# mmSir/SpatioTemporalEntropyModel

Hardware: AMD Instinct MI355X
Metric: frames/s (higher is better)
Workload: dtype f32; 1 GPU; configs[1]: SpatioTemporalPriorModel_Res(256,192) training step on mbt2018(192,192) latents, 16 septuplets x 7 frames x 256x256 per GPU, EMLoss, clip 1.0 + Adam 1e-4 / aux Adam 1e-3; per_gpu_batch=16, global_batch=16, parallelism=dp1, stream_priorities=latents=0,side=-1,compute=-1, stream_cu_masks=latents=block:160, plan_selectors=library defaults

## Files before the change

spatiotemporalentropymodel_amd/_lib.py:

```python
from __future__ import annotations

import ctypes as C
import os

from . import _abi

_PKG = os.path.dirname(os.path.abspath(__file__))
HIP_SO = os.environ.get("STEM_HIP_LIBRARY") or os.path.join(_PKG, "libstem_hip.so")
RANS_SO = os.environ.get("STEM_RANS_LIBRARY") or os.path.join(_PKG, "libstem_rans.so")

DP_SO = os.environ.get("STEM_DP_LIBRARY") or os.path.join(_PKG, "libstem_dp.so")
_hip = None
_rans = None
_dp = None


class StemLibraryError(RuntimeError):
    pass


def _header(name):
    path = os.path.join(_PKG, "..", "include", name)
    if not os.path.exists(path):
        raise StemLibraryError(f"{path} is missing: the ctypes prototypes and structures are read from the C headers")
    return path


def _tables(header):
    protos = _abi.prototypes(_header(header))
    return protos, {n: args for n, (_, args) in protos.items()}, {n: res for n, (res, _) in protos.items() if res is not C.c_int}


_HIP_PROTO, _HIP_SIG, _RESTYPE = _tables("stem_hip.h")
_HIP_BATCH_PROTO, _HIP_BATCH_SIG, _ = _tables("stem_ar_batch.h")
_HIP_BLOCKS_PROTO, _HIP_BLOCKS_SIG, _ = _tables("stem_blocks.h")
_HIP_HYPERPRIOR_PROTO, _HIP_HYPERPRIOR_SIG, _ = _tables("stem_hyperprior.h")
_RANS_PROTO, _RANS_SIG, _RANS_RESTYPE = _tables("stem_rans.h")
_DP_PROTO, _DP_SIG, _ = _tables("stem_dp.h")
_STRUCTS = _abi.structs(_header("stem_hip.h"))


class PackDesc(C.Structure):
    _fields_ = _STRUCTS["stem_pack_desc"]


class F16PackDesc(C.Structure):
    _fields_ = _STRUCTS["stem_f16x2_pack_desc"]


class F16PairDesc(C.Structure):
    _fields_ = _STRUCTS["stem_f16x2_pair_desc"]


class UnpackDesc(C.Structure):
    _fields_ = _STRUCTS["stem_unpack_desc"]


class BiasFinalDesc(C.Structure):
    _fields_ = _STRUCTS["stem_bias_final_desc"]


class WaveSeg(C.Structure):
    _fields_ = _STRUCTS["stem_wave_seg"]


def _bind(lib, protos):
    for name, (restype, argtypes) in protos.items():
        fn = getattr(lib, name)
        fn.argtypes = argtypes
        fn.restype = restype
    return lib


def hip():
    global _hip
    if _hip is None:
        if not os.path.exists(HIP_SO):
            raise StemLibraryError(
                f"{HIP_SO} is missing: build it with `python -c 'import __graft_entry__ as g; g.build()'` "
                "(hipcc --offload-arch=gfx950).  There is no CPU fallback for the STEM kernels.")
        lib = C.CDLL(HIP_SO)
        for protos in (_HIP_PROTO, _HIP_BATCH_PROTO, _HIP_BLOCKS_PROTO, _HIP_HYPERPRIOR_PROTO):
            _bind(lib, protos)
        _hip = lib
    return _hip


def rans():
    global _rans
    if _rans is None:
        if not os.path.exists(RANS_SO):
            raise StemLibraryError(f"{RANS_SO} is missing: run `make -C {os.path.join(_PKG, 'csrc')}`")
        _rans = _bind(C.CDLL(RANS_SO), _RANS_PROTO)
    return _rans


def check(rc: int):
    if rc != 0:
        raise RuntimeError((hip().stem_last_error() or b"").decode() or f"libstem_hip error {rc}")


def declared_hip_symbols():
    return sorted(_HIP_SIG)


# ... 28 lines not shown
```

spatiotemporalentropymodel_amd/csrc/conv_f16x3.hip:

```cpp
#include <math.h>
#include <stdlib.h>

#include <type_traits>

#include "f16x3_layout.h"

namespace {

constexpr int XP = BN + 4;
constexpr int imax(int a, int b) { return a > b ? a : b; }
constexpr int lds_stages(int depth) { return depth == 3 ? 3 : 2; }
constexpr int lds_taps(int bm, int depth) { return imax(imax(lds_stages(depth) * NPL * (bm + BN) * 64, 6 * NPL * bm * 64 + NPL * BN * 64), bm * XP * 4); }
constexpr int lds_total(int bm, int depth) { return lds_taps(bm, depth) + 32 * 4; }

struct Fx3Phase {
    int ntaps, S;
    int dy0, dx0;
    int wofs;
    int cps, nsplit;
    int wsofs;
    int ooy, oox;
};

struct Fx3Args {
// ... 533 lines not shown
            h16x8 h0, h1;
#pragma unroll
            for (int c = 0; c < 4; ++c) {
                hp_t x0, x1;
                q_split(v0[c], oscale, x0, x1);
                h0[c] = x0; h1[c] = x1;
                q_split(v1[c], oscale, x0, x1);
                h0[4 + c] = x0; h1[4 + c] = x1;
            }
            unsigned char *dst = yp + (size_t)m * opix + sl * SLAB + p * 16;
            *reinterpret_cast<h16x8 *>(dst) = h0;
            *reinterpret_cast<h16x8 *>(dst + 64) = h1;
        }
    }
}

enum { GEN_EPI_BIAS = 0, GEN_EPI_LRELU = 1, GEN_EPI_DACT = 2 };

constexpr int GTP = GBN + 4;
constexpr bool GEN_DEFAULT_MFMA16 = true;
constexpr int glds_main(int gbm) { return 2 * NPL * (gbm + GBN) * 64 > gbm * GTP * 4 ? 2 * NPL * (gbm + GBN) * 64 : gbm * GTP * 4; }
constexpr int glds(int gbm) { return glds_main(gbm) + 32 * 4; }

template <int GBM, int MS, bool PH = false>
__global__ __launch_bounds__(GBM * 4, 2) void conv_f16x3_gen_kernel(const Fx3Args a)
{
    static_assert(MS == 32 || MS == 16, "MFMA shape");
    int bxt = blockIdx.x, phase = 0;
    if constexpr (PH) {
        phase = blockIdx.x / a.ptiles;
        bxt = blockIdx.x - phase * a.ptiles;
    }
    const int ntaps = PH ? a.ph[phase].ntaps : a.ntaps, tapS = PH ? a.ph[phase].S : a.S;
    const int cps = PH ? a.ph[phase].cps : a.cps, nsplit = PH ? a.ph[phase].nsplit : a.nsplit;
    const int pdy0 = PH ? a.ph[phase].dy0 : (int)a.dy[0], pdx0 = PH ? a.ph[phase].dx0 : (int)a.dx[0];
    const int wofs = PH ? a.ph[phase].wofs : 0;
    if constexpr (PH) {
        if ((int)blockIdx.z >= nsplit) return;
    }
    float *const wsb = PH ? a.ws + a.ph[phase].wsofs : a.ws;
    constexpr int GNT = GBM * 4, GA_PLANE = GBM * 64, GA_BUF = NPL * GA_PLANE;
    constexpr int PL = NPL, BPC = NPL * GBN * 4 / GNT;
    extern __shared__ __attribute__((aligned(16))) unsigned char smem[];
    unsigned char *As = smem;
    unsigned char *Bs = smem + 2 * GA_BUF;
    int *tapi = reinterpret_cast<int *>(smem + glds_main(GBM));
// ... 188 lines not shown
            step(1, raB, rbB);
            __syncthreads();
        }
        if (q < q_end) {
            step(0, raA, rbA);
            __syncthreads();
        }
    } else {
        int q = q_begin;
        for (; q + 1 < q_end; q += 2) {
            step_dead(0, raA, rbA);
            __syncthreads();
            step_dead(1, raB, rbB);
            __syncthreads();
        }
        if (q < q_end) {
            step_dead(0, raA, rbA);
            __syncthreads();
        }
    }

    float *T = reinterpret_cast<float *>(smem);
    const int Npad = gridDim.y * GBN;
    constexpr int ERS = GNT / 32, ER = GBM / ERS;
    const int ec4 = tid & 31, er0 = tid >> 5;
    f32x4 ev[ER];
    auto OROW = [&](int m) -> size_t {
        if constexpr (!PH) return (size_t)m;
        const int ohw = a.OH * a.OW, b = m / ohw, rem = m - b * ohw, qy = rem / a.OW, qx = rem - qy * a.OW;
        return ((size_t)b * a.OHf + 2 * qy + a.ph[phase].ooy) * a.OWf + 2 * qx + a.ph[phase].oox;
    };
    auto MOK = [&](int m) -> bool {
        if (m >= Mtot) return false;
        if constexpr (!PH) return true;
        const int ohw = a.OH * a.OW, rem = m % ohw, qy = rem / a.OW, qx = rem - qy * a.OW;
        return 2 * qy + a.ph[phase].ooy < a.OHf && 2 * qx + a.ph[phase].oox < a.OWf;
    };
    if (nsplit > 1) {
        float *wsp = wsb + (size_t)zsplit * Mtot * Npad;
#pragma unroll
        for (int j = 0; j < 2; ++j) {
#pragma unroll
            for (int r = 0; r < 16; ++r) {
                const int m = bm0 + ROWL(r), n = bn0 + COLL(j, r);
                if (m < Mtot) __hip_atomic_store(&wsp[(size_t)m * Npad + n], acc[j][r], __ATOMIC_RELAXED, __HIP_MEMORY_SCOPE_AGENT);
            }
        }
        asm volatile("s_waitcnt vmcnt(0)" ::: "memory");
        __syncthreads();
        if (tid == 0) {
            int *c = a.cnt + blockIdx.y * gridDim.x + blockIdx.x;
            tapi[0] = splitk_last_arriver(c, nsplit);
        }
        __syncthreads();
        if (!tapi[0]) return;
        constexpr int SC1 = 16;
        const __amdgpu_buffer_rsrc_t rws = __builtin_amdgcn_make_buffer_rsrc(wsb, 0, (int)((size_t)nsplit * Mtot * Npad * 4), 0x00020000);
        const int sstep = Mtot * Npad * 4;
        int eoff[ER];
#pragma unroll
        for (int k = 0; k < ER; ++k) {
            const int m = bm0 + er0 + ERS * k;
            eoff[k] = m < Mtot ? (m * Npad + bn0 + ec4 * 4) * 4 : OOR;
        }
#pragma unroll
        for (int k = 0; k < ER; ++k) ev[k] = f32x4{0.f, 0.f, 0.f, 0.f};
#pragma unroll
        for (int kb = 0; kb < ER; kb += 4)
            for (int sp = 0; sp < nsplit; sp += 4) {
                f32x4 tt[4][4];
#pragma unroll
                for (int k = 0; k < 4; ++k)
#pragma unroll
                    for (int u = 0; u < 4; ++u)
                        tt[k][u] = __builtin_bit_cast(f32x4, __builtin_amdgcn_raw_buffer_load_b128(rws, sp + u < nsplit ? eoff[kb + k] : OOR,
                                                                                                      (sp + u < nsplit ? sp + u : 0) * sstep, SC1));
#pragma unroll
                for (int k = 0; k < 4; ++k)
#pragma unroll
                    for (int u = 0; u < 4; ++u) ev[kb + k] += tt[k][u];
            }
    } else {
#pragma unroll
        for (int j = 0; j < 2; ++j)
#pragma unroll
            for (int r = 0; r < 16; ++r) T[ROWL(r) * GTP + COLL(j, r)] = acc[j][r];
        __syncthreads();
#pragma unroll
        for (int k = 0; k < ER; ++k) ev[k] = *reinterpret_cast<const f32x4 *>(&T[(er0 + ERS * k) * GTP + ec4 * 4]);
    }
    float omax = 0.f;
    const int ecol = bn0 + ec4 * 4;
    const bool colok = ecol < a.N;
    f32x4 ebias = {0.f, 0.f, 0.f, 0.f};
    if (a.bias && colok) {
#pragma unroll
        for (int c = 0; c < 4; ++c) ebias[c] = a.bias[ecol + c];
    }
    f32x4 ez[ER];
    if (a.epi == GEN_EPI_DACT) {
#pragma unroll
        for (int k = 0; k < ER; ++k) {
            const int m = bm0 + er0 + ERS * k;
            ez[k] = (colok && MOK(m)) ? *reinterpret_cast<const f32x4 *>(a.z + OROW(m) * a.ldz + ecol) : f32x4{1.f, 1.f, 1.f, 1.f};
        }
    }
#pragma unroll
    for (int k = 0; k < ER; ++k) {
        const int row = er0 + ERS * k, m = bm0 + row;
        f32x4 v = ev[k] * fac + ebias;
        if (a.epi == GEN_EPI_LRELU) {
#pragma unroll
            for (int c = 0; c < 4; ++c) v[c] = v[c] > 0.f ? v[c] : v[c] * a.slope;
        } else if (a.epi == GEN_EPI_DACT) {
#pragma unroll
            for (int c = 0; c < 4; ++c) v[c] = ez[k][c] > 0.f ? v[c] : v[c] * a.slope;
        }
        if (colok && MOK(m)) {
            if (a.y) *reinterpret_cast<f32x4 *>(a.y + OROW(m) * a.ldy + ecol) = v;
            omax = fmaxf(fmaxf(omax, fmaxf(fabsf(v[0]), fabsf(v[1]))), fmaxf(fabsf(v[2]), fabsf(v[3])));
        }
        if (a.yp) *reinterpret_cast<f32x4 *>(&T[row * GTP + ec4 * 4]) = v;
    }
    if (a.yq) {
        omax = block_max(omax, qred);
        if (tid == 0) {
            a.yq[QREC_HDR + blockIdx.y * gridDim.x + blockIdx.x] = omax;
            if (blockIdx.x == 0 && blockIdx.y == 0) {
                q_header(a.yq, gridDim.x * gridDim.y);
                if (!a.yp) a.yq[1] = 1.f;
            }
        }
    }
    if (a.yp) {
        __syncthreads();
        const int oslab = a.N / KC, opix = oslab * SLAB;
        unsigned char *yp = static_cast<unsigned char *>(a.yp);
        for (int e = tid; e < GBM * (GBN / 8); e += GNT) {
            const int row = e / (GBN / 8), c8 = e - row * (GBN / 8);
            const int m = bm0 + row, n = bn0 + c8 * 8;
            if (!MOK(m) || n >= a.N) continue;
            const f32x4 v0 = *reinterpret_cast<const f32x4 *>(&T[row * GTP + c8 * 8]);
            const f32x4 v1 = *reinterpret_cast<const f32x4 *>(&T[row * GTP + c8 * 8 + 4]);
            h16x8 h0, h1;
#pragma unroll
            for (int c = 0; c < 4; ++c) {
                hp_t x0, x1;
                q_split(v0[c], oscale, x0, x1);
                h0[c] = x0; h1[c] = x1;
                q_split(v1[c], oscale, x0, x1);
                h0[4 + c] = x0; h1[4 + c] = x1;
            }
            unsigned char *dst = yp + OROW(m) * opix + (n >> 5) * SLAB + ((n >> 3) & 3) * 16;
            *reinterpret_cast<h16x8 *>(dst) = h0;
            *reinterpret_cast<h16x8 *>(dst + 64) = h1;
        }
    }
}

}

static int conv2d_f16x3_launch(const void *xp, const float *xq, const void *wp, const float *bias, const float *beta, const void *gp,
                                float beta_min, int act, float slope, float *y, int ldy, void *yp, float *yq, int B, int H, int W, int C, int N,
                                int R, int S, int stride, int pad, void *stream);

STEM_EXPORT int stem_conv2d_f16x3_fwd(const void *xp, const float *xq, const void *wp, const float *bias, const float *beta, const void *gp,
                                       float beta_min, float *y, int ldy, void *yp, float *yq, int B, int H, int W, int C, int N, int R, int S,
                                       int stride, int pad, void *stream)
{
    return conv2d_f16x3_launch(xp, xq, wp, bias, beta, gp, beta_min, 0, 0.f, y, ldy, yp, yq, B, H, W, C, N, R, S, stride, pad, stream);
}

STEM_EXPORT int stem_conv2d_f16x3_fwd_act(const void *xp, const float *xq, const void *wp, const float *bias, int act, float slope, float *y, int ldy,
                                           void *yp, float *yq, int B, int H, int W, int C, int N, int R, int S, int stride, int pad, void *stream)
{
    STEM_CHECK_ARG(act == 0 || act == 1, "stem_conv2d_f16x3_fwd_act: act is 0 (none) or 1 (leaky ReLU with `slope`)");
    STEM_CHECK_ARG(!act || fabsf(slope) <= 1.f, "stem_conv2d_f16x3_fwd_act: |slope| <= 1");
    return conv2d_f16x3_launch(xp, xq, wp, bias, nullptr, nullptr, 1e-6f, act, slope, y, ldy, yp, yq, B, H, W, C, N, R, S, stride, pad, stream);
}

// ... 73 lines not shown
    const int forced = stem_tuning(STEM_TUNE_FX3_SPLIT);
    if (forced > 0) return forced < nchunks ? forced : nchunks;
    if (nchunks <= 40 && tiles >= 128) return 1;
    int best = 1;
    double best_cost = 1e30;
    for (int s = 1; s <= 16 && s * 8 <= nchunks; ++s) {
        const int cps = cdiv(nchunks, s), ns = cdiv(nchunks, cps), rounds = cdiv(tiles * ns, 256);
        const double cost = rounds * (cps + 6.0) * (rounds == 1 ? 1.67 : 1.0) + (ns > 1 ? 0.3 * ns : 0.0);
        if (cost < best_cost - 1e-9) {
            best_cost = cost;
            best = ns;
        }
    }
    return best;
}

int gen_bm(int M, int ntn, int nchunks)
{
    const int forced = stem_tuning(STEM_TUNE_FX3_GEN_TILE);
    if (forced) return forced;
    (void)nchunks;
    return cdiv(M, 128) * ntn >= 64 ? 128 : 64;
}
}

STEM_EXPORT size_t stem_conv2d_f16x3_gen_workspace_bytes(int B, int H, int W, int C, int N, int R, int S, int stride, int pad, int taps)
{
    const int OH = (H + 2 * pad - R) / stride + 1, OW = (W + 2 * pad - S) / stride + 1;
    if (OH < 1 || OW < 1 || C % 32) return 0;
    const int M = B * OH * OW, nchunks = (C / 32) * (taps > 0 ? taps : R * S), tiles = cdiv(M, gen_bm(M, cdiv(N, GBN), nchunks)) * cdiv(N, GBN);
    int s = gen_split(tiles, nchunks);
    if (stem_fx3_img_eligible(B, H, W, N, R, S, stride, pad)) {
        const int si = stem_fx3_img_split(stem_fx3_img_tiles(B, H, W, N), nchunks);
        if (si > s) s = si;
    }
    while (s > 1 && (size_t)s * M * cdiv(N, GBN) * GBN * sizeof(float) >= 0x7FFFFF00ull) --s;
    return s > 1 ? kGenCntBytes + (size_t)s * M * cdiv(N, GBN) * GBN * sizeof(float) : 0;
}

STEM_EXPORT int stem_conv2d_f16x3_gen_fwd(const void *xp, const float *xq, int xpix, const void *wp, const float *bias, int epi, float slope,
                                           const float *z, int ldz, float *y, int ldy, void *yp, float *yq, int B, int H, int W, int C, int N, int R,
                                           int S, int stride, int pad, int taps, void *ws, size_t ws_bytes, void *stream)
{
    STEM_CHECK_ARG(taps >= 0 && taps <= R * S, "stem_conv2d_f16x3_gen_fwd: 0 <= taps <= R*S (taps=%d)", taps);
    const int T = taps > 0 ? taps : R * S;
    STEM_CHECK_ARG(xp && xq && wp && (y || yp) && (yq || !yp), "stem_conv2d_f16x3_gen_fwd: null pointer (planes come with their scale records)");
    STEM_CHECK_ARG(epi == GEN_EPI_BIAS || fabsf(slope) <= 1.f, "stem_conv2d_f16x3_gen_fwd: |slope| <= 1");
    STEM_CHECK_ARG(B >= 1 && H >= 1 && W >= 1 && C >= 32 && C % 32 == 0 && N >= 4 && N % 4 == 0 && R >= 1 && S >= 1 && R * S <= MAXTAP &&
                   stride >= 1 && pad >= 0, "stem_conv2d_f16x3_gen_fwd: C %% 32 == 0, N %% 4 == 0, R*S <= %d (C=%d N=%d R=%d S=%d)", MAXTAP, C, N, R, S);
    STEM_CHECK_ARG(!yp || N % 32 == 0, "stem_conv2d_f16x3_gen_fwd: planes output needs N %% 32 == 0 (N=%d)", N);
    STEM_CHECK_ARG(!y || (ldy >= N && ldy % 4 == 0 && ((uintptr_t)y & 15) == 0), "stem_conv2d_f16x3_gen_fwd: y rows must be 16-byte aligned, ldy >= N");
    STEM_CHECK_ARG(epi >= GEN_EPI_BIAS && epi <= GEN_EPI_DACT, "stem_conv2d_f16x3_gen_fwd: unknown epilogue %d", epi);
    STEM_CHECK_ARG(epi != GEN_EPI_DACT || (z && ldz >= N && ldz % 4 == 0 && ((uintptr_t)z & 15) == 0), "stem_conv2d_f16x3_gen_fwd: DACT needs z (16-byte aligned rows)");
    const int OH = (H + 2 * pad - R) / stride + 1, OW = (W + 2 * pad - S) / stride + 1;
    STEM_CHECK_ARG(OH >= 1 && OW >= 1, "stem_conv2d_f16x3_gen_fwd: empty output");
    if (xpix == 0) xpix = (C / 32) * SLAB;
    STEM_CHECK_ARG(xpix >= (C / 32) * SLAB && xpix % SLAB == 0, "stem_conv2d_f16x3_gen_fwd: xpix must be a multiple of %d bytes covering C channels", SLAB);
    const size_t xb = (size_t)B * H * W * xpix, wb = gen_image_bytes(N, C, R, S);
    const int M = B * OH * OW, ntn = cdiv(N, GBN), nchunks = (C / 32) * T, bm = gen_bm(M, ntn, nchunks), tiles = cdiv(M, bm) * ntn;
    STEM_CHECK_ARG(xb < 0x7FFFFF00ull && wb < 0x7FFFFF00ull && (size_t)M * ntn * GBN * 4 < 0x7FFFFF00ull,
                   "stem_conv2d_f16x3_gen_fwd: operand views must stay below 2 GiB (split the batch)");
    Fx3Args a;
    memset(&a, 0, sizeof(a));
    a.xp = xp; a.wp = wp; a.bias = bias; a.y = y; a.yp = yp; a.ldy = ldy; a.z = z; a.ldz = ldz; a.epi = epi; a.slope = slope;
    const float *wq = reinterpret_cast<const float *>(static_cast<const unsigned char *>(wp) + wb);
    a.xq = xq; a.yq = yq; a.wq = wq;
    a.B = B; a.H = H; a.W = W; a.C = C; a.N = N; a.OH = OH; a.OW = OW; a.stride = stride; a.ntaps = T; a.S = S;
    a.xbytes = (int)xb; a.wbytes = (int)wb; a.xpix = xpix;
    for (int r = 0; r < R; ++r)
        for (int s = 0; s < S; ++s) {
            a.dy[r * S + s] = (signed char)(r - pad);
            a.dx[r * S + s] = (signed char)(s - pad);
        }
    const bool img = stem_fx3_img_eligible(B, H, W, N, R, S, stride, pad);
    const int itiles = img ? stem_fx3_img_tiles(B, H, W, N) : 0;
    int split = img ? stem_fx3_img_split(itiles, nchunks) : gen_split(tiles, nchunks);
    while (split > 1 && (size_t)split * M * ntn * GBN * sizeof(float) >= 0x7FFFFF00ull) --split;
    const size_t need = kGenCntBytes + (size_t)split * M * ntn * GBN * sizeof(float);
    if (split > 1 && (!ws || ws_bytes < need || (size_t)tiles * sizeof(int) > kGenCntBytes)) split = 1;
    if (img)
        return stem_fx3_img_launch(xp, xq, xpix, (int)xb, wp, wq, (int)wb,
                                   bias, epi, slope, z, ldz, y, ldy, yp, yq, B, H, W, C, N, R, T, split,
                                   split > 1 ? reinterpret_cast<float *>(static_cast<unsigned char *>(ws) + kGenCntBytes) : nullptr,
                                   split > 1 ? static_cast<int *>(ws) : nullptr, stream);
    a.nsplit = split;
    a.cps = cdiv(nchunks, split);
    a.nsplit = cdiv(nchunks, a.cps);
    if (a.nsplit > 1) {
        a.cnt = static_cast<int *>(ws);
        a.ws = reinterpret_cast<float *>(static_cast<unsigned char *>(ws) + kGenCntBytes);
    }
    static bool attr_done = false;
    if (!attr_done) {
        (void)hipFuncSetAttribute((const void *)conv_f16x3_gen_kernel<64, 32>, hipFuncAttributeMaxDynamicSharedMemorySize, glds(64));
        (void)hipFuncSetAttribute((const void *)conv_f16x3_gen_kernel<128, 32>, hipFuncAttributeMaxDynamicSharedMemorySize, glds(128));
        (void)hipFuncSetAttribute((const void *)conv_f16x3_gen_kernel<64, 16>, hipFuncAttributeMaxDynamicSharedMemorySize, glds(64));
        (void)hipFuncSetAttribute((const void *)conv_f16x3_gen_kernel<128, 16>, hipFuncAttributeMaxDynamicSharedMemorySize, glds(128));
        attr_done = true;
    }
    const dim3 grid(cdiv(M, bm), ntn, a.nsplit);
    const int gmsel = stem_tuning(STEM_TUNE_FX3_GEN_MFMA);
    const bool g16 = gmsel ? gmsel == 16 : GEN_DEFAULT_MFMA16;
    if (bm == 128 && g16)
        hipLaunchKernelGGL((conv_f16x3_gen_kernel<128, 16>), grid, dim3(512), glds(128), (hipStream_t)stream, a);
    else if (bm == 128)
        hipLaunchKernelGGL((conv_f16x3_gen_kernel<128, 32>), grid, dim3(512), glds(128), (hipStream_t)stream, a);
    else if (g16)
        hipLaunchKernelGGL((conv_f16x3_gen_kernel<64, 16>), grid, dim3(256), glds(64), (hipStream_t)stream, a);
    else
        hipLaunchKernelGGL((conv_f16x3_gen_kernel<64, 32>), grid, dim3(256), glds(64), (hipStream_t)stream, a);
    STEM_LAUNCH_CHECK("stem_conv2d_f16x3_gen_fwd");
    return 0;
}

namespace {
int tconv_cps(int tiles_per_phase, const int (&nchunks)[4])
{
    const int forced = stem_tuning(STEM_TUNE_FX3_SPLIT);
    int maxc = 0;
    for (int p = 0; p < 4; ++p) maxc = nchunks[p] > maxc ? nchunks[p] : maxc;
    if (forced > 0) return cdiv(maxc, forced < maxc ? forced : maxc);
    if (stem_tuning(STEM_TUNE_TCONV_CPS) > 0) return stem_tuning(STEM_TUNE_TCONV_CPS);
    for (int cps = 12; cps < maxc; ++cps) {
        int wgs = 0, maxns = 0;
        for (int p = 0; p < 4; ++p) {
            const int ns = cdiv(nchunks[p], cps);
// ... 99 lines not shown
```

spatiotemporalentropymodel_amd/csrc/pack.hip:

```cpp
#include <stdarg.h>

#include "stem_common.h"

static thread_local char g_err[512] = "";
void stem_set_error(const char *fmt, ...)
{
    va_list ap;
    va_start(ap, fmt);
    vsnprintf(g_err, sizeof(g_err), fmt, ap);
    va_end(ap);
}
STEM_EXPORT const char *stem_last_error(void) { return g_err; }
STEM_EXPORT int stem_abi_version(void) { return 5; }

static int g_tuning[STEM_TUNE_COUNT] = {0};
static const char *const kTuningNames[STEM_TUNE_COUNT] = {"fx3_tile", "fx3_split", "wg3_split", "arp_workers", "fx3_depth", "fx3_gen_tile", "fx3_mfma", "fx3_gen_mfma", "fx3_gen_img", "fx3_img_w", "wg3_row", "wg3_minch", "tconv_cps", "arp_giveup_at", "unpack_mb"};
int stem_tuning(int id) { return g_tuning[id]; }
STEM_EXPORT int stem_tuning_set(const char *name, int value)
{
    STEM_CHECK_ARG(name && value >= 0, "stem_tuning_set: null name or negative value");
    for (int i = 0; i < STEM_TUNE_COUNT; ++i)
        if (!strcmp(name, kTuningNames[i])) {
            STEM_CHECK_ARG(i != STEM_TUNE_FX3_TILE || value == 0 || value == 64 || value == 128, "stem_tuning_set: fx3_tile is 0 (automatic), 64 or 128");
            STEM_CHECK_ARG(i != STEM_TUNE_FX3_GEN_TILE || value == 0 || value == 64 || value == 128, "stem_tuning_set: fx3_gen_tile is 0 (automatic), 64 or 128");
            STEM_CHECK_ARG(i != STEM_TUNE_FX3_DEPTH || value == 0 || value == 2 || value == 3, "stem_tuning_set: fx3_depth is 0 (automatic), 2 or 3 (LDS stages of the split-operand main loops)");
            STEM_CHECK_ARG(i != STEM_TUNE_FX3_GEN_MFMA || value == 0 || value == 16 || value == 32, "stem_tuning_set: fx3_gen_mfma is 0 (automatic), 16 or 32 (rows of the general kernel's MFMA shape)");
            STEM_CHECK_ARG(i != STEM_TUNE_UNPACK_MB || value == 0 || (value % 32 == 0 && value >= 32 && value <= 192), "stem_tuning_set: unpack_mb is 0 (automatic) or a multiple of 32 up to 192");
            STEM_CHECK_ARG(i != STEM_TUNE_FX3_MFMA || value == 0 || value == 16 || value == 32, "stem_tuning_set: fx3_mfma is 0 (automatic), 16 or 32 (rows of the MFMA shape)");
            g_tuning[i] = value;
            return 0;
        }
    stem_set_error("stem_tuning_set: unknown selector '%s' (fx3_tile, fx3_split, wg3_split, arp_workers, fx3_depth, fx3_gen_tile, fx3_mfma, fx3_gen_mfma, fx3_gen_img, fx3_img_w, wg3_row, wg3_minch, tconv_cps, arp_giveup_at, unpack_mb)", name);
    return -1;
}
STEM_EXPORT int stem_tuning_get(const char *name)
{
    for (int i = 0; name && i < STEM_TUNE_COUNT; ++i)
        if (!strcmp(name, kTuningNames[i])) return g_tuning[i];
    return -1;
}

namespace {

__global__ __launch_bounds__(256) void pack_kernel(float *w, float *out, int A, int Bd, int T, long sa, long sb,
                                                   int R, int S, int masked)
{
    extern __shared__ float tile[];
    const int a = blockIdx.x;
    const int n = Bd * T;
    for (int i = threadIdx.x; i < n; i += 256) {
        const int b = i / T, t = i - b * T;
        float v = w[a * sa + b * sb + t];
        if (masked & 3) {
            const int r = t / S, s = t - r * S;
            if (r > R / 2 || (r == R / 2 && s >= S / 2 + ((masked >> 2) & 1))) {
// ... 419 lines not shown
```

spatiotemporalentropymodel_amd/csrc/stem_common.h:

```cpp
#pragma once
#include <hip/hip_runtime.h>
#include <stdint.h>
#include <stdio.h>
#include <string.h>

#include "../../include/stem_hip.h"

#define STEM_EXPORT extern "C" __attribute__((visibility("default")))

void stem_set_error(const char *fmt, ...);

#define STEM_CHECK_ARG(cond, ...)        \
    do {                                 \
        if (!(cond)) {                   \
            stem_set_error(__VA_ARGS__); \
            return -1;                   \
        }                                \
    } while (0)

#define STEM_LAUNCH_CHECK(name)                                                         \
    do {                                                                                \
        hipError_t e_ = hipGetLastError();                                              \
        if (e_ != hipSuccess) {                                                         \
            stem_set_error("%s: launch failed: %s", name, hipGetErrorString(e_));       \
            return -2;                                                                  \
        }                                                                               \
    } while (0)

typedef float f32x4 __attribute__((ext_vector_type(4)));
typedef float f32x16 __attribute__((ext_vector_type(16)));

static inline int cdiv(int a, int b) { return (a + b - 1) / b; }
static inline size_t cdivz(size_t a, size_t b) { return (a + b - 1) / b; }

enum { STEM_TUNE_FX3_TILE = 0, STEM_TUNE_FX3_SPLIT, STEM_TUNE_WG3_SPLIT, STEM_TUNE_ARP_WORKERS, STEM_TUNE_FX3_DEPTH, STEM_TUNE_FX3_GEN_TILE, STEM_TUNE_FX3_MFMA, STEM_TUNE_FX3_GEN_MFMA, STEM_TUNE_FX3_GEN_IMG, STEM_TUNE_FX3_IMG_W, STEM_TUNE_WG3_ROW, STEM_TUNE_WG3_MINCH, STEM_TUNE_TCONV_CPS, STEM_TUNE_ARP_GIVEUP_AT, STEM_TUNE_UNPACK_MB, STEM_TUNE_COUNT };
int stem_tuning(int id);
bool stem_fx3_img_eligible(int B, int H, int W, int N, int R, int S, int stride, int pad);
int stem_fx3_img_tiles(int B, int H, int W, int N);
int stem_fx3_img_split(int tiles, int nchunks);
int stem_fx3_img_launch(const void *xp, const float *xq, int xpix, int xbytes, const void *wp, const float *wq, int wbytes, const float *bias, int epi,
                        float slope, const float *z, int ldz, float *y, int ldy, void *yp, float *yq, int B, int H, int W, int C, int N, int KS,
                        int T, int split, float *ws, int *cnt, void *stream);

#define STEM_ADAM_CHUNK 4096

typedef _Float16 hp_t;
typedef hp_t hp8 __attribute__((ext_vector_type(8)));
#define STEM_MFMA16(a, b, c) __builtin_amdgcn_mfma_f32_32x32x16_f16(a, b, c, 0, 0, 0)

constexpr int QREC_HDR = 16;
#ifdef __HIPCC__
__device__ inline int q_nslots(const float *q) { return reinterpret_cast<const int *>(q)[0]; }
__device__ inline float q_inv(const float *q) { return q[1]; }
__device__ inline void q_header(float *q, int n)
{
    reinterpret_cast<int *>(q)[0] = n;
#pragma unroll
    for (int i = 2; i < QREC_HDR; ++i) q[i] = 0.f;
// ... 66 lines not shown
```

Baseline: 10020 frames/s.

## Add pointwise 1x1 conv kernel with four-stage LDS ring and plan selector

Adds a dedicated 1x1, stride-1 kernel for the f16x3 general convolution. It streams activation and weight chunks through a four-slot LDS ring using buffer-to-LDS loads, and uses hand-scheduled 16x16x32 MFMA interleaving with explicit waitcnt and barrier control. The epilogue is factored into shared helpers, and plan selection moves into a gen_plan function that is exported and gated by a new fx3_gen_pw tuning selector. The aim is to hide load latency for pointwise convolutions. The trade-off is a larger LDS footprint, which can lower occupancy, plus more complex synchronisation.

```diff
diff --git a/include/stem_plan.h b/include/stem_plan.h
--- /dev/null
+++ b/include/stem_plan.h
@@ -0,0 +1,16 @@
+#ifndef STEM_PLAN_H
+#define STEM_PLAN_H
+
+#include <stddef.h>
+
+#ifdef __cplusplus
+extern "C" {
+#endif
+
+int stem_conv2d_f16x3_gen_plan(int B, int H, int W, int C, int N, int R, int S, int stride, int pad, int taps, size_t ws_bytes, int *split);
+
+#ifdef __cplusplus
+}
+#endif
+
+#endif
diff --git a/spatiotemporalentropymodel_amd/_lib.py b/spatiotemporalentropymodel_amd/_lib.py
--- a/spatiotemporalentropymodel_amd/_lib.py
+++ b/spatiotemporalentropymodel_amd/_lib.py
@@ -35,6 +35,7 @@
 _HIP_BATCH_PROTO, _HIP_BATCH_SIG, _ = _tables("stem_ar_batch.h")
 _HIP_BLOCKS_PROTO, _HIP_BLOCKS_SIG, _ = _tables("stem_blocks.h")
 _HIP_HYPERPRIOR_PROTO, _HIP_HYPERPRIOR_SIG, _ = _tables("stem_hyperprior.h")
+_HIP_PLAN_PROTO, _HIP_PLAN_SIG, _ = _tables("stem_plan.h")
 _RANS_PROTO, _RANS_SIG, _RANS_RESTYPE = _tables("stem_rans.h")
 _DP_PROTO, _DP_SIG, _ = _tables("stem_dp.h")
 _STRUCTS = _abi.structs(_header("stem_hip.h"))
@@ -80,7 +81,7 @@
                 f"{HIP_SO} is missing: build it with `python -c 'import __graft_entry__ as g; g.build()'` "
                 "(hipcc --offload-arch=gfx950).  There is no CPU fallback for the STEM kernels.")
         lib = C.CDLL(HIP_SO)
-        for protos in (_HIP_PROTO, _HIP_BATCH_PROTO, _HIP_BLOCKS_PROTO, _HIP_HYPERPRIOR_PROTO):
+        for protos in (_HIP_PROTO, _HIP_BATCH_PROTO, _HIP_BLOCKS_PROTO, _HIP_HYPERPRIOR_PROTO, _HIP_PLAN_PROTO):
             _bind(lib, protos)
         _hip = lib
     return _hip
diff --git a/spatiotemporalentropymodel_amd/csrc/conv_f16x3.hip b/spatiotemporalentropymodel_amd/csrc/conv_f16x3.hip
--- a/spatiotemporalentropymodel_amd/csrc/conv_f16x3.hip
+++ b/spatiotemporalentropymodel_amd/csrc/conv_f16x3.hip
@@ -579,6 +579,109 @@
 constexpr int glds_main(int gbm) { return 2 * NPL * (gbm + GBN) * 64 > gbm * GTP * 4 ? 2 * NPL * (gbm + GBN) * 64 : gbm * GTP * 4; }
 constexpr int glds(int gbm) { return glds_main(gbm) + 32 * 4; }
 
+constexpr int GEN_ER = 8;
+template <int GBM, typename TPos>
+__device__ __forceinline__ void gen_park(float *T, TPos tpos, const f32x16 (&acc)[2], f32x4 (&ev)[GEN_ER])
+{
+    constexpr int ERS = GBM * 4 / 32;
+    const int tid = threadIdx.x, ec4 = tid & 31, er0 = tid >> 5;
+#pragma unroll
+    for (int j = 0; j < 2; ++j)
+#pragma unroll
+        for (int r = 0; r < 16; ++r) T[tpos(j, r)] = acc[j][r];
+    __syncthreads();
+#pragma unroll
+    for (int k = 0; k < GEN_ER; ++k) ev[k] = *reinterpret_cast<const f32x4 *>(&T[(er0 + ERS * k) * GTP + ec4 * 4]);
+}
+
+template <int GBM, bool PH>
+__device__ __forceinline__ void gen_epilogue(const Fx3Args &a, const int phase, const int bm0, const int bn0, const float fac, const float oscale,
+                                             float *T, float *qred, const f32x4 (&ev)[GEN_ER])
+{
+    constexpr int GNT = GBM * 4, ERS = GNT / 32, ER = GEN_ER;
+    static_assert(ER * ERS == GBM, "eight pieces per thread");
+    const int tid = threadIdx.x, ec4 = tid & 31, er0 = tid >> 5;
+    const int Mtot = a.B * a.OH * a.OW;
+    auto OROW = [&](int m) -> size_t {
+        if constexpr (!PH) return (size_t)m;
+        const int ohw = a.OH * a.OW, b = m / ohw, rem = m - b * ohw, qy = rem / a.OW, qx = rem - qy * a.OW;
+        return ((size_t)b * a.OHf + 2 * qy + a.ph[phase].ooy) * a.OWf + 2 * qx + a.ph[phase].oox;
+    };
+    auto MOK = [&](int m) -> bool {
+        if (m >= Mtot) return false;
+        if constexpr (!PH) return true;
+        const int ohw = a.OH * a.OW, rem = m % ohw, qy = rem / a.OW, qx = rem - qy * a.OW;
+        return 2 * qy + a.ph[phase].ooy < a.OHf && 2 * qx + a.ph[phase].oox < a.OWf;
+    };
+    float omax = 0.f;
+    const int ecol = bn0 + ec4 * 4;
+    const bool colok = ecol < a.N;
+    f32x4 ebias = {0.f, 0.f, 0.f, 0.f};
+    if (a.bias && colok) {
+#pragma unroll
+        for (int c = 0; c < 4; ++c) ebias[c] = a.bias[ecol + c];
+    }
+    f32x4 ez[ER];
+    if (a.epi == GEN_EPI_DACT) {
+#pragma unroll
+        for (int k = 0; k < ER; ++k) {
+            const int m = bm0 + er0 + ERS * k;
+            ez[k] = (colok && MOK(m)) ? *reinterpret_cast<const f32x4 *>(a.z + OROW(m) * a.ldz + ecol) : f32x4{1.f, 1.f, 1.f, 1.f};
+        }
+    }
+#pragma unroll
+    for (int k = 0; k < ER; ++k) {
+        const int row = er0 + ERS * k, m = bm0 + row;
+        f32x4 v = ev[k] * fac + ebias;
+        if (a.epi == GEN_EPI_LRELU) {
+#pragma unroll
+            for (int c = 0; c < 4; ++c) v[c] = v[c] > 0.f ? v[c] : v[c] * a.slope;
+        } else if (a.epi == GEN_EPI_DACT) {
+#pragma unroll
+            for (int c = 0; c < 4; ++c) v[c] = ez[k][c] > 0.f ? v[c] : v[c] * a.slope;
+        }
+        if (colok && MOK(m)) {
+            if (a.y) *reinterpret_cast<f32x4 *>(a.y + OROW(m) * a.ldy + ecol) = v;
+            omax = fmaxf(fmaxf(omax, fmaxf(fabsf(v[0]), fabsf(v[1]))), fmaxf(fabsf(v[2]), fabsf(v[3])));
+        }
+        if (a.yp) *reinterpret_cast<f32x4 *>(&T[row * GTP + ec4 * 4]) = v;
+    }
+    if (a.yq) {
+        omax = block_max(omax, qred);
+        if (tid == 0) {
+            a.yq[QREC_HDR + blockIdx.y * gridDim.x + blockIdx.x] = omax;
+            if (blockIdx.x == 0 && blockIdx.y == 0) {
+                q_header(a.yq, gridDim.x * gridDim.y);
+                if (!a.yp) a.yq[1] = 1.f;
+            }
+        }
+    }
+    if (a.yp) {
+        __syncthreads();
+        const int oslab = a.N / KC, opix = oslab * SLAB;
+        unsigned char *yp = static_cast<unsigned char *>(a.yp);
+        for (int e = tid; e < GBM * (GBN / 8); e += GNT) {
+            const int row = e / (GBN / 8), c8 = e - row * (GBN / 8);
+            const int m = bm0 + row, n = bn0 + c8 * 8;
+            if (!MOK(m) || n >= a.N) continue;
+            const f32x4 v0 = *reinterpret_cast<const f32x4 *>(&T[row * GTP + c8 * 8]);
+            const f32x4 v1 = *reinterpret_cast<const f32x4 *>(&T[row * GTP + c8 * 8 + 4]);
+            h16x8 h0, h1;
+#pragma unroll
+            for (int c = 0; c < 4; ++c) {
+                hp_t x0, x1;
+                q_split(v0[c], oscale, x0, x1);
+                h0[c] = x0; h1[c] = x1;
+                q_split(v1[c], oscale, x0, x1);
+                h0[4 + c] = x0; h1[4 + c] = x1;
+            }
+            unsigned char *dst = yp + OROW(m) * opix + (n >> 5) * SLAB + ((n >> 3) & 3) * 16;
+            *reinterpret_cast<h16x8 *>(dst) = h0;
+            *reinterpret_cast<h16x8 *>(dst + 64) = h1;
+        }
+    }
+}
+
 template <int GBM, int MS, bool PH = false>
 __global__ __launch_bounds__(GBM * 4, 2) void conv_f16x3_gen_kernel(const Fx3Args a)
 {
@@ -813,20 +916,9 @@
 
     float *T = reinterpret_cast<float *>(smem);
     const int Npad = gridDim.y * GBN;
-    constexpr int ERS = GNT / 32, ER = GBM / ERS;
+    constexpr int ERS = GNT / 32, ER = GEN_ER;
     const int ec4 = tid & 31, er0 = tid >> 5;
     f32x4 ev[ER];
-    auto OROW = [&](int m) -> size_t {
-        if constexpr (!PH) return (size_t)m;
-        const int ohw = a.OH * a.OW, b = m / ohw, rem = m - b * ohw, qy = rem / a.OW, qx = rem - qy * a.OW;
-        return ((size_t)b * a.OHf + 2 * qy + a.ph[phase].ooy) * a.OWf + 2 * qx + a.ph[phase].oox;
-    };
-    auto MOK = [&](int m) -> bool {
-        if (m >= Mtot) return false;
-        if constexpr (!PH) return true;
-        const int ohw = a.OH * a.OW, rem = m % ohw, qy = rem / a.OW, qx = rem - qy * a.OW;
-        return 2 * qy + a.ph[phase].ooy < a.OHf && 2 * qx + a.ph[phase].oox < a.OWf;
-    };
     if (nsplit > 1) {
         float *wsp = wsb + (size_t)zsplit * Mtot * Npad;
 #pragma unroll
@@ -872,81 +964,164 @@
                     for (int u = 0; u < 4; ++u) ev[kb + k] += tt[k][u];
             }
     } else {
-#pragma unroll
-        for (int j = 0; j < 2; ++j)
-#pragma unroll
-            for (int r = 0; r < 16; ++r) T[ROWL(r) * GTP + COLL(j, r)] = acc[j][r];
-        __syncthreads();
-#pragma unroll
-        for (int k = 0; k < ER; ++k) ev[k] = *reinterpret_cast<const f32x4 *>(&T[(er0 + ERS * k) * GTP + ec4 * 4]);
-    }
-    float omax = 0.f;
-    const int ecol = bn0 + ec4 * 4;
-    const bool colok = ecol < a.N;
-    f32x4 ebias = {0.f, 0.f, 0.f, 0.f};
-    if (a.bias && colok) {
-#pragma unroll
-        for (int c = 0; c < 4; ++c) ebias[c] = a.bias[ecol + c];
-    }
-    f32x4 ez[ER];
-    if (a.epi == GEN_EPI_DACT) {
-#pragma unroll
-        for (int k = 0; k < ER; ++k) {
-            const int m = bm0 + er0 + ERS * k;
-            ez[k] = (colok && MOK(m)) ? *reinterpret_cast<const f32x4 *>(a.z + OROW(m) * a.ldz + ecol) : f32x4{1.f, 1.f, 1.f, 1.f};
-        }
-    }
-#pragma unroll
-    for (int k = 0; k < ER; ++k) {
-        const int row = er0 + ERS * k, m = bm0 + row;
-        f32x4 v = ev[k] * fac + ebias;
-        if (a.epi == GEN_EPI_LRELU) {
-#pragma unroll
-            for (int c = 0; c < 4; ++c) v[c] = v[c] > 0.f ? v[c] : v[c] * a.slope;
-        } else if (a.epi == GEN_EPI_DACT) {
-#pragma unroll
-            for (int c = 0; c < 4; ++c) v[c] = ez[k][c] > 0.f ? v[c] : v[c] * a.slope;
-        }
-        if (colok && MOK(m)) {
-            if (a.y) *reinterpret_cast<f32x4 *>(a.y + OROW(m) * a.ldy + ecol) = v;
-            omax = fmaxf(fmaxf(omax, fmaxf(fabsf(v[0]), fabsf(v[1]))), fmaxf(fabsf(v[2]), fabsf(v[3])));
-        }
-        if (a.yp) *reinterpret_cast<f32x4 *>(&T[row * GTP + ec4 * 4]) = v;
-    }
-    if (a.yq) {
-        omax = block_max(omax, qred);
-        if (tid == 0) {
-            a.yq[QREC_HDR + blockIdx.y * gridDim.x + blockIdx.x] = omax;
-            if (blockIdx.x == 0 && blockIdx.y == 0) {
-                q_header(a.yq, gridDim.x * gridDim.y);
-                if (!a.yp) a.yq[1] = 1.f;
-            }
-        }
-    }
+        gen_park<GBM>(T, [&](int j, int r) { return ROWL(r) * GTP + COLL(j, r); }, acc, ev);
+    }
+    gen_epilogue<GBM, PH>(a, phase, bm0, bn0, fac, oscale, T, qred, ev);
+}
+
+constexpr int PW_RING = 4;
+constexpr int pw_stage(int gbm) { return NPL * (gbm + GBN) * 64; }
+constexpr int pw_lds_main(int gbm) { return PW_RING * pw_stage(gbm) > gbm * GTP * 4 ? PW_RING * pw_stage(gbm) : gbm * GTP * 4; }
+constexpr int pw_lds(int gbm) { return pw_lds_main(gbm) + 32 * 4; }
+
+template <int GBM>
+__global__ __launch_bounds__(GBM * 4) void conv_f16x3_pw_kernel(const Fx3Args a)
+{
+    constexpr int GNT = GBM * 4, NW = GNT / 64, GA_PLANE = GBM * 64, GA_BUF = NPL * GA_PLANE, STAGE = pw_stage(GBM);
+    constexpr int PL = NPL;
+    constexpr int BW = GB_BUF / NW, BI = BW / 1024;
+    constexpr int PW_PER = PL + BI;
+    static_assert(GBM / 16 == NW, "one 16-row piece of each activation plane per wavefront");
+    extern __shared__ __attribute__((aligned(16))) unsigned char smem[];
+    float *qred = reinterpret_cast<float *>(smem + pw_lds_main(GBM));
+
+    const int tid = threadIdx.x, lane = tid & 63, wave = __builtin_amdgcn_readfirstlane(tid >> 6);
+    const int Mtot = a.B * a.OH * a.OW;
+    const int bm0 = blockIdx.x * GBM, bn0 = blockIdx.y * GBN;
+    const int nchunks = a.C / KC, q_last = nchunks - 1;
+    const int wbase = blockIdx.y * nchunks;
+
+    const __amdgpu_buffer_rsrc_t rx = __builtin_amdgcn_make_buffer_rsrc(const_cast<void *>(a.xp), 0, a.xbytes, 0x00020000);
+    const __amdgpu_buffer_rsrc_t rw = __builtin_amdgcn_make_buffer_rsrc(const_cast<void *>(a.wp), 0, a.wbytes, 0x00020000);
+    int va;
+    {
+        const int row = wave * 16 + (lane >> 2), m = bm0 + row;
+        va = m < Mtot ? m * a.xpix + (((lane & 3) ^ ((row >> 2) & 3)) << 4) : OOR;
+    }
+    const int vb = wave * BW + lane * 16;
+    auto dma = [&](int q, int slot) {
+        q = q < q_last ? q : q_last;
+        unsigned char *st = smem + slot * STAGE;
+        const int sA = q * SLAB, sB = (wbase + q) * GB_BUF;
+#pragma unroll
+        for (int pl = 0; pl < PL; ++pl)
+            __builtin_amdgcn_raw_ptr_buffer_load_lds(rx, (__attribute__((address_space(3))) void *)(st + pl * GA_PLANE + wave * 1024), 16, va + pl * PLANE1, sA, 0, 0);
+        auto *lb = (__attribute__((address_space(3))) void *)(st + GA_BUF + wave * BW);
+        __builtin_amdgcn_raw_ptr_buffer_load_lds(rw, lb, 16, vb, sB, 0, 0);
+        __builtin_amdgcn_raw_ptr_buffer_load_lds(rw, lb, 16, vb, sB, 1024, 0);
+        if constexpr (BI == 4) {
+            __builtin_amdgcn_raw_ptr_buffer_load_lds(rw, lb, 16, vb, sB, 2048, 0);
+            __builtin_amdgcn_raw_ptr_buffer_load_lds(rw, lb, 16, vb, sB, 3072, 0);
+        }
+    };
+
+    const int wm0 = (wave >> 1) * 32, wn0 = (wave & 1) * 64;
+    const int l16 = lane & 15, lq = lane >> 4;
+    const int cm = 4 * pi4(l16 >> 2) + (l16 & 3), rq = 4 * pi4(lq);
+    const int rdA16 = (wm0 + cm) * 64 + ((lq ^ pi4(l16 >> 2)) << 4), rdB16 = GA_BUF + (wn0 + cm) * 64 + ((lq ^ pi4(l16 >> 2)) << 4);
+    auto ROWL = [&](int r) { return wm0 + ((r >> 2) & 1) * 16 + rq + (r & 3); };
+    auto COLL = [&](int j, int r) { return wn0 + j * 32 + (r >> 3) * 16 + cm; };
+    f32x4 a16[2][4];
+#pragma unroll
+    for (int mi = 0; mi < 2; ++mi)
+#pragma unroll
+        for (int nj = 0; nj < 4; ++nj) a16[mi][nj] = f32x4{0.f, 0.f, 0.f, 0.f};
+    auto rdfrag = [&](int slot, h16x8 (&A)[2][PL], h16x8 (&B)[4][PL]) {
+        const unsigned char *st = smem + slot * STAGE;
+#pragma unroll
+        for (int mi = 0; mi < 2; ++mi)
+#pragma unroll
+            for (int pl = 0; pl < PL; ++pl) A[mi][pl] = *reinterpret_cast<const h16x8 *>(st + rdA16 + mi * 16 * 64 + pl * GA_PLANE);
+#pragma unroll
+        for (int nj = 0; nj < 4; ++nj)
+#pragma unroll
+            for (int pl = 0; pl < PL; ++pl) B[nj][pl] = *reinterpret_cast<const h16x8 *>(st + rdB16 + nj * 16 * 64 + pl * GB_PLANE);
+    };
+    auto mma = [&](const h16x8 (&A)[2][PL], const h16x8 (&B)[4][PL]) {
+#pragma unroll
+        for (int prod = 0; prod < 3; ++prod)
+#pragma unroll
+            for (int nj = 0; nj < 4; ++nj)
+#pragma unroll
+                for (int mi = 0; mi < 2; ++mi)
+                    a16[mi][nj] = __builtin_amdgcn_mfma_f32_16x16x32_f16(A[mi][prod == 0 ? 1 : 0], B[nj][prod == 1 ? 1 : 0], a16[mi][nj], 0, 0, 0);
+    };
+
+    dma(0, 0);
+    dma(1, 1);
+    dma(2, 2);
+    dma(3, 3);
+    const float fac = q_inv(a.xq) * q_inv(a.wq);
+    float oscale = 1.f;
     if (a.yp) {
-        __syncthreads();
-        const int oslab = a.N / KC, opix = oslab * SLAB;
-        unsigned char *yp = static_cast<unsigned char *>(a.yp);
-        for (int e = tid; e < GBM * (GBN / 8); e += GNT) {
-            const int row = e / (GBN / 8), c8 = e - row * (GBN / 8);
-            const int m = bm0 + row, n = bn0 + c8 * 8;
-            if (!MOK(m) || n >= a.N) continue;
-            const f32x4 v0 = *reinterpret_cast<const f32x4 *>(&T[row * GTP + c8 * 8]);
-            const f32x4 v1 = *reinterpret_cast<const f32x4 *>(&T[row * GTP + c8 * 8 + 4]);
-            h16x8 h0, h1;
-#pragma unroll
-            for (int c = 0; c < 4; ++c) {
-                hp_t x0, x1;
-                q_split(v0[c], oscale, x0, x1);
-                h0[c] = x0; h1[c] = x1;
-                q_split(v1[c], oscale, x0, x1);
-                h0[4 + c] = x0; h1[4 + c] = x1;
-            }
-            unsigned char *dst = yp + OROW(m) * opix + (n >> 5) * SLAB + ((n >> 3) & 3) * 16;
-            *reinterpret_cast<h16x8 *>(dst) = h0;
-            *reinterpret_cast<h16x8 *>(dst + 64) = h1;
-        }
-    }
+        const float xmax = q_amax(a.xq, qred), wmax = q_amax(a.wq, qred);
+        float bm = 0.f;
+        if (a.bias)
+            for (int n = tid; n < a.N; n += GNT) bm = fmaxf(bm, fabsf(a.bias[n]));
+        bm = block_max(bm, qred);
+        const int oe = q_exp((float)a.C * xmax * wmax + bm);
+        oscale = q_pow2(oe);
+        if (blockIdx.x == 0 && blockIdx.y == 0 && tid == 0) a.yq[1] = q_pow2(-oe);
+    }
+    const bool dead = bn0 + wn0 >= a.N;
+    auto run = [&](auto live_tag) {
+        constexpr bool LIVE = decltype(live_tag)::value;
+        h16x8 A0[2][PL], B0[4][PL], A1[2][PL], B1[4][PL];
+        asm volatile("s_waitcnt vmcnt(%0)" ::"n"(3 * PW_PER) : "memory");
+        __builtin_amdgcn_sched_barrier(0);
+        __builtin_amdgcn_s_waitcnt(0xC07F);
+        __builtin_amdgcn_sched_barrier(0);
+        asm volatile("s_barrier" ::: "memory");
+        if constexpr (LIVE) rdfrag(0, A0, B0);
+        auto chunk = [&](int c, h16x8 (&Ac)[2][PL], h16x8 (&Bc)[4][PL], h16x8 (&An)[2][PL], h16x8 (&Bn)[4][PL]) {
+            __builtin_amdgcn_sched_barrier(0);
+            __builtin_amdgcn_s_waitcnt(0xC07F);
+            __builtin_amdgcn_sched_barrier(0);
+            asm volatile("s_waitcnt vmcnt(%0)\n\ts_barrier" ::"n"(2 * PW_PER) : "memory");
+            __builtin_amdgcn_sched_barrier(0);
+            if constexpr (LIVE) {
+                rdfrag((c + 1) & (PW_RING - 1), An, Bn);
+                mma(Ac, Bc);
+                dma(c + 4, c & (PW_RING - 1));
+#pragma unroll
+                for (int i = 0; i < 12; ++i) {
+                    __builtin_amdgcn_sched_group_barrier(0x008, 1, 0);
+                    __builtin_amdgcn_sched_group_barrier(0x100, 1, 0);
+                }
+#pragma unroll
+                for (int i = 0; i < PW_PER; ++i) {
+                    __builtin_amdgcn_sched_group_barrier(0x008, 12 / PW_PER, 0);
+                    __builtin_amdgcn_sched_group_barrier(0x020, 1, 0);
+                }
+            } else {
+                dma(c + 4, c & (PW_RING - 1));
+            }
+            __builtin_amdgcn_sched_barrier(0);
+        };
+        int c = 0;
+#pragma unroll 1
+        for (; c + 1 < nchunks; c += 2) {
+            chunk(c, A0, B0, A1, B1);
+            chunk(c + 1, A1, B1, A0, B0);
+        }
+        if (c < nchunks) chunk(c, A0, B0, A1, B1);
+    };
+    if (dead)
+        run(std::false_type{});
+    else
+        run(std::true_type{});
+    asm volatile("s_waitcnt vmcnt(0)" ::: "memory");
+    __syncthreads();
+
+    f32x16 acc[2];
+#pragma unroll
+    for (int j = 0; j < 2; ++j)
+#pragma unroll
+        for (int r = 0; r < 16; ++r) acc[j][r] = a16[(r >> 2) & 1][2 * j + (r >> 3)][r & 3];
+    f32x4 ev[GEN_ER];
+    float *T = reinterpret_cast<float *>(smem);
+    gen_park<GBM>(T, [&](int j, int r) { return ROWL(r) * GTP + COLL(j, r); }, acc, ev);
+    gen_epilogue<GBM, false>(a, 0, bm0, bn0, fac, oscale, T, qred, ev);
 }
 
 }
@@ -1066,6 +1241,46 @@
     (void)nchunks;
     return cdiv(M, 128) * ntn >= 64 ? 128 : 64;
 }
+
+bool gen_pw(int M, int N, int C, int bm)
+{
+    const int forced = stem_tuning(STEM_TUNE_FX3_GEN_PW);
+    if (forced) return forced == 1;
+    (void)M; (void)N; (void)C; (void)bm;
+    return true;
+}
+
+struct GenPlan {
+    int img, split, cps, bm, pw;
+};
+GenPlan gen_plan(int B, int H, int W, int C, int N, int R, int S, int stride, int pad, int T, bool have_ws, size_t ws_bytes)
+{
+    const int OH = (H + 2 * pad - R) / stride + 1, OW = (W + 2 * pad - S) / stride + 1;
+    const int M = B * OH * OW, ntn = cdiv(N, GBN), nchunks = (C / 32) * T, bm = gen_bm(M, ntn, nchunks), tiles = cdiv(M, bm) * ntn;
+    GenPlan p;
+    p.img = stem_fx3_img_eligible(B, H, W, N, R, S, stride, pad) ? 1 : 0;
+    p.bm = bm;
+    int split = p.img ? stem_fx3_img_split(stem_fx3_img_tiles(B, H, W, N), nchunks) : gen_split(tiles, nchunks);
+    while (split > 1 && (size_t)split * M * ntn * GBN * sizeof(float) >= 0x7FFFFF00ull) --split;
+    const size_t need = kGenCntBytes + (size_t)split * M * ntn * GBN * sizeof(float);
+    if (split > 1 && (!have_ws || ws_bytes < need || (size_t)tiles * sizeof(int) > kGenCntBytes)) split = 1;
+    p.cps = cdiv(nchunks, split);
+    if (!p.img) split = cdiv(nchunks, p.cps);
+    p.split = split;
+    const int gmsel = stem_tuning(STEM_TUNE_FX3_GEN_MFMA);
+    const bool g16 = gmsel ? gmsel == 16 : GEN_DEFAULT_MFMA16;
+    p.pw = !p.img && split == 1 && g16 && R == 1 && S == 1 && T == 1 && stride == 1 && pad == 0 && gen_pw(M, N, C, bm) ? 1 : 0;
+    return p;
+}
+}
+
+STEM_EXPORT int stem_conv2d_f16x3_gen_plan(int B, int H, int W, int C, int N, int R, int S, int stride, int pad, int taps, size_t ws_bytes, int *split)
+{
+    if (B < 1 || H < 1 || W < 1 || C < 32 || C % 32 || N < 4 || R < 1 || S < 1 || R * S > MAXTAP || stride < 1 || pad < 0 || taps < 0 || taps > R * S) return -1;
+    if ((H + 2 * pad - R) / stride + 1 < 1 || (W + 2 * pad - S) / stride + 1 < 1) return -1;
+    const GenPlan p = gen_plan(B, H, W, C, N, R, S, stride, pad, taps > 0 ? taps : R * S, ws_bytes > 0, ws_bytes);
+    if (split) *split = p.split;
+    return p.img ? 1 : (p.pw ? 2 : 0);
 }
 
 STEM_EXPORT size_t stem_conv2d_f16x3_gen_workspace_bytes(int B, int H, int W, int C, int N, int R, int S, int stride, int pad, int taps)
@@ -1101,7 +1316,7 @@
     if (xpix == 0) xpix = (C / 32) * SLAB;
     STEM_CHECK_ARG(xpix >= (C / 32) * SLAB && xpix % SLAB == 0, "stem_conv2d_f16x3_gen_fwd: xpix must be a multiple of %d bytes covering C channels", SLAB);
     const size_t xb = (size_t)B * H * W * xpix, wb = gen_image_bytes(N, C, R, S);
-    const int M = B * OH * OW, ntn = cdiv(N, GBN), nchunks = (C / 32) * T, bm = gen_bm(M, ntn, nchunks), tiles = cdiv(M, bm) * ntn;
+    const int M = B * OH * OW, ntn = cdiv(N, GBN);
     STEM_CHECK_ARG(xb < 0x7FFFFF00ull && wb < 0x7FFFFF00ull && (size_t)M * ntn * GBN * 4 < 0x7FFFFF00ull,
                    "stem_conv2d_f16x3_gen_fwd: operand views must stay below 2 GiB (split the batch)");
     Fx3Args a;
@@ -1116,20 +1331,15 @@
             a.dy[r * S + s] = (signed char)(r - pad);
             a.dx[r * S + s] = (signed char)(s - pad);
         }
-    const bool img = stem_fx3_img_eligible(B, H, W, N, R, S, stride, pad);
-    const int itiles = img ? stem_fx3_img_tiles(B, H, W, N) : 0;
-    int split = img ? stem_fx3_img_split(itiles, nchunks) : gen_split(tiles, nchunks);
-    while (split > 1 && (size_t)split * M * ntn * GBN * sizeof(float) >= 0x7FFFFF00ull) --split;
-    const size_t need = kGenCntBytes + (size_t)split * M * ntn * GBN * sizeof(float);
-    if (split > 1 && (!ws || ws_bytes < need || (size_t)tiles * sizeof(int) > kGenCntBytes)) split = 1;
-    if (img)
+    const GenPlan plan = gen_plan(B, H, W, C, N, R, S, stride, pad, T, ws != nullptr, ws_bytes);
+    const int split = plan.split, bm = plan.bm;
+    if (plan.img)
         return stem_fx3_img_launch(xp, xq, xpix, (int)xb, wp, wq, (int)wb,
                                    bias, epi, slope, z, ldz, y, ldy, yp, yq, B, H, W, C, N, R, T, split,
                                    split > 1 ? reinterpret_cast<float *>(static_cast<unsigned char *>(ws) + kGenCntBytes) : nullptr,
                                    split > 1 ? static_cast<int *>(ws) : nullptr, stream);
+    a.cps = plan.cps;
     a.nsplit = split;
-    a.cps = cdiv(nchunks, split);
-    a.nsplit = cdiv(nchunks, a.cps);
     if (a.nsplit > 1) {
         a.cnt = static_cast<int *>(ws);
         a.ws = reinterpret_cast<float *>(static_cast<unsigned char *>(ws) + kGenCntBytes);
@@ -1140,12 +1350,18 @@
         (void)hipFuncSetAttribute((const void *)conv_f16x3_gen_kernel<128, 32>, hipFuncAttributeMaxDynamicSharedMemorySize, glds(128));
         (void)hipFuncSetAttribute((const void *)conv_f16x3_gen_kernel<64, 16>, hipFuncAttributeMaxDynamicSharedMemorySize, glds(64));
         (void)hipFuncSetAttribute((const void *)conv_f16x3_gen_kernel<128, 16>, hipFuncAttributeMaxDynamicSharedMemorySize, glds(128));
+        (void)hipFuncSetAttribute((const void *)conv_f16x3_pw_kernel<64>, hipFuncAttributeMaxDynamicSharedMemorySize, pw_lds(64));
+        (void)hipFuncSetAttribute((const void *)conv_f16x3_pw_kernel<128>, hipFuncAttributeMaxDynamicSharedMemorySize, pw_lds(128));
         attr_done = true;
     }
     const dim3 grid(cdiv(M, bm), ntn, a.nsplit);
     const int gmsel = stem_tuning(STEM_TUNE_FX3_GEN_MFMA);
     const bool g16 = gmsel ? gmsel == 16 : GEN_DEFAULT_MFMA16;
-    if (bm == 128 && g16)
+    if (plan.pw && bm == 128)
+        hipLaunchKernelGGL((conv_f16x3_pw_kernel<128>), grid, dim3(512), pw_lds(128), (hipStream_t)stream, a);
+    else if (plan.pw)
+        hipLaunchKernelGGL((conv_f16x3_pw_kernel<64>), grid, dim3(256), pw_lds(64), (hipStream_t)stream, a);
+    else if (bm == 128 && g16)
         hipLaunchKernelGGL((conv_f16x3_gen_kernel<128, 16>), grid, dim3(512), glds(128), (hipStream_t)stream, a);
     else if (bm == 128)
         hipLaunchKernelGGL((conv_f16x3_gen_kernel<128, 32>), grid, dim3(512), glds(128), (hipStream_t)stream, a);
diff --git a/spatiotemporalentropymodel_amd/csrc/pack.hip b/spatiotemporalentropymodel_amd/csrc/pack.hip
--- a/spatiotemporalentropymodel_amd/csrc/pack.hip
+++ b/spatiotemporalentropymodel_amd/csrc/pack.hip
@@ -14,7 +14,7 @@
 STEM_EXPORT int stem_abi_version(void) { return 5; }
 
 static int g_tuning[STEM_TUNE_COUNT] = {0};
-static const char *const kTuningNames[STEM_TUNE_COUNT] = {"fx3_tile", "fx3_split", "wg3_split", "arp_workers", "fx3_depth", "fx3_gen_tile", "fx3_mfma", "fx3_gen_mfma", "fx3_gen_img", "fx3_img_w", "wg3_row", "wg3_minch", "tconv_cps", "arp_giveup_at", "unpack_mb"};
+static const char *const kTuningNames[STEM_TUNE_COUNT] = {"fx3_tile", "fx3_split", "wg3_split", "arp_workers", "fx3_depth", "fx3_gen_tile", "fx3_mfma", "fx3_gen_mfma", "fx3_gen_img", "fx3_img_w", "wg3_row", "wg3_minch", "tconv_cps", "arp_giveup_at", "unpack_mb", "fx3_gen_pw"};
 int stem_tuning(int id) { return g_tuning[id]; }
 STEM_EXPORT int stem_tuning_set(const char *name, int value)
 {
@@ -26,11 +26,12 @@
             STEM_CHECK_ARG(i != STEM_TUNE_FX3_DEPTH || value == 0 || value == 2 || value == 3, "stem_tuning_set: fx3_depth is 0 (automatic), 2 or 3 (LDS stages of the split-operand main loops)");
             STEM_CHECK_ARG(i != STEM_TUNE_FX3_GEN_MFMA || value == 0 || value == 16 || value == 32, "stem_tuning_set: fx3_gen_mfma is 0 (automatic), 16 or 32 (rows of the general kernel's MFMA shape)");
             STEM_CHECK_ARG(i != STEM_TUNE_UNPACK_MB || value == 0 || (value % 32 == 0 && value >= 32 && value <= 192), "stem_tuning_set: unpack_mb is 0 (automatic) or a multiple of 32 up to 192");
+            STEM_CHECK_ARG(i != STEM_TUNE_FX3_GEN_PW || value <= 2, "stem_tuning_set: fx3_gen_pw is 0 (automatic), 1 (the pointwise form of the general kernel wherever eligible) or 2 (never)");
             STEM_CHECK_ARG(i != STEM_TUNE_FX3_MFMA || value == 0 || value == 16 || value == 32, "stem_tuning_set: fx3_mfma is 0 (automatic), 16 or 32 (rows of the MFMA shape)");
             g_tuning[i] = value;
             return 0;
         }
-    stem_set_error("stem_tuning_set: unknown selector '%s' (fx3_tile, fx3_split, wg3_split, arp_workers, fx3_depth, fx3_gen_tile, fx3_mfma, fx3_gen_mfma, fx3_gen_img, fx3_img_w, wg3_row, wg3_minch, tconv_cps, arp_giveup_at, unpack_mb)", name);
+    stem_set_error("stem_tuning_set: unknown selector '%s' (fx3_tile, fx3_split, wg3_split, arp_workers, fx3_depth, fx3_gen_tile, fx3_mfma, fx3_gen_mfma, fx3_gen_img, fx3_img_w, wg3_row, wg3_minch, tconv_cps, arp_giveup_at, unpack_mb, fx3_gen_pw)", name);
     return -1;
 }
 STEM_EXPORT int stem_tuning_get(const char *name)
diff --git a/spatiotemporalentropymodel_amd/csrc/stem_common.h b/spatiotemporalentropymodel_amd/csrc/stem_common.h
--- a/spatiotemporalentropymodel_amd/csrc/stem_common.h
+++ b/spatiotemporalentropymodel_amd/csrc/stem_common.h
@@ -33,7 +33,7 @@
 static inline int cdiv(int a, int b) { return (a + b - 1) / b; }
 static inline size_t cdivz(size_t a, size_t b) { return (a + b - 1) / b; }
 
-enum { STEM_TUNE_FX3_TILE = 0, STEM_TUNE_FX3_SPLIT, STEM_TUNE_WG3_SPLIT, STEM_TUNE_ARP_WORKERS, STEM_TUNE_FX3_DEPTH, STEM_TUNE_FX3_GEN_TILE, STEM_TUNE_FX3_MFMA, STEM_TUNE_FX3_GEN_MFMA, STEM_TUNE_FX3_GEN_IMG, STEM_TUNE_FX3_IMG_W, STEM_TUNE_WG3_ROW, STEM_TUNE_WG3_MINCH, STEM_TUNE_TCONV_CPS, STEM_TUNE_ARP_GIVEUP_AT, STEM_TUNE_UNPACK_MB, STEM_TUNE_COUNT };
+enum { STEM_TUNE_FX3_TILE = 0, STEM_TUNE_FX3_SPLIT, STEM_TUNE_WG3_SPLIT, STEM_TUNE_ARP_WORKERS, STEM_TUNE_FX3_DEPTH, STEM_TUNE_FX3_GEN_TILE, STEM_TUNE_FX3_MFMA, STEM_TUNE_FX3_GEN_MFMA, STEM_TUNE_FX3_GEN_IMG, STEM_TUNE_FX3_IMG_W, STEM_TUNE_WG3_ROW, STEM_TUNE_WG3_MINCH, STEM_TUNE_TCONV_CPS, STEM_TUNE_ARP_GIVEUP_AT, STEM_TUNE_UNPACK_MB, STEM_TUNE_FX3_GEN_PW, STEM_TUNE_COUNT };
 int stem_tuning(int id);
 bool stem_fx3_img_eligible(int B, int H, int W, int N, int R, int S, int stride, int pad);
 int stem_fx3_img_tiles(int B, int H, int W, int N);
```

Measured after the change: 9891 frames/s. 0.987x the previous value.
